# AIRI-Institute/nablaDFT

Measured on AMD Instinct MI355X. Metric: conformer-steps/sec (fwd+bwd) + MAE(E,F) vs CPU reference, higher is better.
Workload: dtype f32 (dense products >= 192 tiles: f32 values split exactly into 3 bf16 pieces, 6 MFMA piece products, f32 accumulate; non-finite operands give NaN where plain f32 gives inf); 1 GPU; PaiNN-OC (nablaDFT/painn_pyg, config/model/painn-oc.yaml: F=128 L=6 R=100 rc=5A K=100) energy+forces train step incl. neighbour list, L1+L2 loss, grad all-reduce, clip 5.0, AdamW lr 5e-4; synthetic ~42-atom drug-like conformers, 2048 conformers/GPU/step; conformers_per_gpu=2048, edges_last_step=1737976, parallelism=dp1

## Files before the change

### nabladft_amd/csrc/engine.hip

```cpp
#include <stdarg.h>
#include <stdlib.h>
#include <string.h>

#include "../../include/nablaq.h"
#include "common.h"

thread_local char nq_err_buf[512] = "";
int nq_fail(int code, const char* fmt, ...) {
  va_list ap;
  va_start(ap, fmt);
  vsnprintf(nq_err_buf, sizeof(nq_err_buf), fmt, ap);
  va_end(ap);
  return code;
}

#include <map>
#include <mutex>
#include <utility>
static std::mutex g_lds_mu;
static std::map<std::pair<int, const void*>, size_t> g_lds_granted;
int nq_dyn_lds(const void* kernel, size_t bytes) {
  int dev = 0;
  NQ_HIP(hipGetDevice(&dev));
  std::lock_guard<std::mutex> lock(g_lds_mu);
// ... 110 lines not shown
  W->GXH = take(2 * N * 3 * F); W->GH = take(2 * N * F);
  W->GBR = take(N * 3 * F);
  W->GPHI2 = take(2 * E * 3 * F);
  W->GEDGE = take((F / 64) * E * 4);
  W->GZO = take(2 * N * H); W->TMPW = take(N * H);
  W->GRHO = take(c->rbf_type ? 2 * E * R : 0); W->BCON = take(c->rbf_type ? E * R : 0);
  W->ROWCTR = take(5 * L * NQ_ROWCTR_INTS);
  W->SCHED = take(W->fused ? nq_molgw_sched_ints((int)E, (int)B) : 0);
  W->GWREC = take(W->fused ? nq_molgw_rec_floats((int)E, (int)B) : 0);
  W->GWPART = take(W->fused ? nq_molgw_part_floats((int)F, (int)B) : 0);
  size_t s = 0;
  auto mx = [&](size_t v) { if (v > s) s = v; };
  mx(nq_gemm_tn_scratch_floats(2 * N, 3 * F, F)); mx(nq_gemm_tn_scratch_floats(2 * N, F, 2 * F)); mx(nq_gemm_tn_scratch_floats(6 * N, 2 * F, F));
  mx(W->fused ? nq_gwr_scratch_floats((int)E, (int)F, (int)R) : nq_gemm_tn_scratch_floats(2 * E, 3 * F, R));
  if (W->fused) mx(nq_k0_sort_scratch_ints((int)E, (int)R));
  mx(nq_gemm_tn_scratch_floats(2 * N, F, F)); mx(nq_gemm_tn_scratch_floats(2 * N, H, F));
  mx(nq_colsum_scratch_floats(N > E ? N : E, 3 * F));
  if (c->rbf_type) { mx(nq_colsum_scratch_floats(E, R)); mx(nq_colsum_scratch_floats(E * R, 1)); }
  mx(nq_embed_grad_scratch_floats((int)N, (int)F, (int)T));
  W->scratch_floats = s;
  W->scratch = take(s);
  W->total_floats = o;
  (void)B;
}

enum { GW_PAIR_ROWS = 0, GW_MOLECULE = 1, GW_MIXED = 2 };
struct StepPlan {
  bool fused;
  int gw_mode, gw_cap;
  bool lite;
  bool fused_update;
  bool layer0;
  bool top_layer;
};
static StepPlan plan_step(const nq_painn_cfg* c, const nq_graph* g, bool want_forces) {
  auto env_on = [](const char* name) { const char* v = getenv(name); return v && v[0] == '1'; };
  StepPlan p{};
  p.fused = c->rbf_type == 0 && nq_filter_fits_lds(c->hidden_channels, c->num_rbf) && !env_on("NQ_NO_FUSED_FILTER");
  const char* cap = getenv("NQ_MOLGW_CAP");
  const int hw = nq_molgw_max_atoms();
  p.gw_cap = cap && atoi(cap) > 0 && atoi(cap) < hw ? atoi(cap) : hw;
  p.gw_mode = GW_PAIR_ROWS;
  if (p.fused && !env_on("NQ_NO_MOLGW") && nq_molgw_config_ok(c->hidden_channels, c->num_rbf) && g->max_mol_atoms > 0 && (env_on("NQ_MOLGW") || g->N >= 4096))
    p.gw_mode = g->max_mol_atoms <= p.gw_cap ? GW_MOLECULE : GW_MIXED;
  p.lite = p.fused && want_forces && !env_on("NQ_NO_LITE");
  p.fused_update = nq_updfuse_frag_floats(c->hidden_channels) > 0 && !env_on("NQ_NO_FUSED_UPDATE") && !nq_gemm_exact_f32_requested();
  p.layer0 = !env_on("NQ_NO_LAYER0");
  p.top_layer = !env_on("NQ_NO_TOPLAYER");
  return p;
}
static bool plan_fused(const nq_painn_cfg* c, int32_t N, int32_t E, int32_t B) {
  nq_graph g{};
  g.N = N; g.E = E; g.B = B;
  return plan_step(c, &g, false).fused;
}

struct StepRecord { nq_painn_cfg cfg; int32_t N, E, B, max_mol_atoms; StepPlan plan; };
static std::mutex g_plan_mu;
static std::map<const void*, StepRecord> g_plans;
static StepRecord g_last_plan;
static bool g_have_last_plan = false;
static void record_plan(const void* ws, const nq_painn_cfg* c, const nq_graph* g, const StepPlan& p) {
  std::lock_guard<std::mutex> lock(g_plan_mu);
  g_plans[ws] = StepRecord{*c, g->N, g->E, g->B, g->max_mol_atoms, p};
  g_last_plan = g_plans[ws]; g_have_last_plan = true;
}
static bool last_plan_for(const nq_painn_cfg* c, int32_t N, int32_t E, int32_t B, StepPlan* p) {
  std::lock_guard<std::mutex> lock(g_plan_mu);
  if (!g_have_last_plan || memcmp(&g_last_plan.cfg, c, sizeof(nq_painn_cfg)) != 0 || g_last_plan.N != N || g_last_plan.E != E || g_last_plan.B != B) return false;
  *p = g_last_plan.plan;
  return true;
}
static int recall_plan(const void* ws, const nq_painn_cfg* c, const nq_graph* g, StepPlan* p) {
  std::lock_guard<std::mutex> lock(g_plan_mu);
  auto it = g_plans.find(ws);
  if (it == g_plans.end()) return nq_fail(NQ_ERR_ARG, "nq_painn_backward: no forward call has prepared this workspace");
  const StepRecord& r = it->second;
  if (memcmp(&r.cfg, c, sizeof(nq_painn_cfg)) != 0 || r.N != g->N || r.E != g->E || r.B != g->B || r.max_mol_atoms != g->max_mol_atoms)
    return nq_fail(NQ_ERR_ARG, "nq_painn_backward: the last forward call on this workspace was made for a different model or batch");
  *p = r.plan;
  return NQ_OK;
}

static NqGraphView view_of(const nq_graph* g) {
  NqGraphView v;
  v.N = g->N; v.B = g->B; v.E = g->E;
  v.mol_ptr = g->mol_ptr; v.row_ptr = g->row_ptr; v.col = g->col; v.rev = g->rev;
  v.geom = reinterpret_cast<const float4*>(g->geom); v.z = g->z; v.atom_mol = g->atom_mol; v.lowptr = g->lowptr;
  return v;
}

static int check_common(const nq_painn_cfg* cfg, const nq_graph* g, const void* ws, size_t ws_bytes, bool fused, WsLayout* W, ParamLayout* P) {
  if (!cfg || !g || !ws) return nq_fail(NQ_ERR_ARG, "null argument");
  NQ_TRY(make_param_layout(cfg, P));
  if (g->N <= 0 || g->B <= 0) return nq_fail(NQ_ERR_ARG, "empty batch");
  if (g->E <= 0) return nq_fail(NQ_ERR_NO_EDGES, "batch has no edges within the cutoff");
  if ((reinterpret_cast<uintptr_t>(ws) & 15) != 0) return nq_fail(NQ_ERR_ARG, "workspace must be 16-byte aligned");
  make_ws_layout(cfg, g->N, g->E, g->B, fused, W);
  if (cfg->filter_mode != 0 && cfg->filter_mode != 1) return nq_fail(NQ_ERR_ARG, "filter_mode must be 0 (painn_pyg) or 1 (schnetpack)");
  if (cfg->filter_mode == 1 && !W->fused)
    return nq_fail(NQ_ERR_ARG, "filter_mode 1 (schnetpack) needs the fused-filter path: hidden_channels in {64,128,256} and WrT fitting the LDS");
  if (ws_bytes < W->total_floats * sizeof(float))
    return nq_fail(NQ_ERR_WORKSPACE, "workspace too small: %zu < %zu bytes", ws_bytes, W->total_floats * sizeof(float));
  return NQ_OK;
}

extern "C" {

int nq_abi_version(void) { return NQ_ABI_VERSION; }
int32_t nq_painn_molecule_lds_atoms(void) { return nq_molgw_max_atoms(); }

void nq_profile_enable(int32_t on) { nq_profile_on = on; }
int nq_profile_read2(char* names, int32_t name_stride, double* total_ms, int64_t* counts, double* flops, int32_t cap) {
  (void)hipDeviceSynchronize();
  std::vector<double> tot(g_prof_names.size(), 0.0), fl(g_prof_names.size(), 0.0);
  std::vector<long long> cnt(g_prof_names.size(), 0);
  for (auto& r : g_prof_recs) {
    float ms = 0.f;
    if (hipEventElapsedTime(&ms, r.a, r.b) == hipSuccess) { tot[r.name_id] += ms; cnt[r.name_id] += 1; fl[r.name_id] += r.flops; }
    (void)hipEventDestroy(r.a); (void)hipEventDestroy(r.b);
  }
  g_prof_recs.clear();
  int n = (int)g_prof_names.size();
  for (int i = 0; i < n && i < cap; ++i) {
    snprintf(names + (size_t)i * name_stride, name_stride, "%s", g_prof_names[i].c_str());
    total_ms[i] = tot[i]; counts[i] = cnt[i];
    if (flops) flops[i] = fl[i];
  }
  return n;
}
int nq_profile_read(char* names, int32_t name_stride, double* total_ms, int64_t* counts, int32_t cap) {
  return nq_profile_read2(names, name_stride, total_ms, counts, nullptr, cap);
}
const char* nq_last_error(void) { return nq_err_buf; }

int nq_graph_count(const float* pos, const int32_t* mol_ptr, int32_t N, int32_t B, int32_t max_mol_atoms, double cutoff,
                   int32_t max_neighbors, int32_t* deg, int32_t* lowdeg, int32_t* row_ptr, int32_t* lowptr, int32_t* E_host, void* stream) {
// ... 100 lines not shown
  else if (!strcmp(name, "e_atom")) { base = tangent ? W.te_atom : W.e_atom; rows = n; w = 1; dual = false; tangent = 0; }
  else if (!strcmp(name, "t_d")) { base = W.TD; rows = e; w = 1; dual = false; }
  else if (!strcmp(name, "t_r")) { base = W.TR; rows = e; w = 3; dual = false; }
  else if (!strcmp(name, "gedge")) { base = W.GEDGE; rows = (F / 64) * e; w = 4; dual = false; }
  else return nq_fail(NQ_ERR_ARG, "unknown workspace buffer '%s'", name);
#undef LAYER_OK
  if (tangent && !dual) return nq_fail(NQ_ERR_ARG, "buffer '%s' has no tangent half", name);
  *off = base + (tangent ? rows * w : 0);
  *count = rows * w;
  return NQ_OK;
}

int nq_painn_forward(const nq_painn_cfg* cfg, const float* params, const float* rbf_offsets, const nq_graph* graph, void* workspace,
                     size_t workspace_bytes, float* energy, float* forces, void* stream) {
  if (!cfg || !graph) return nq_fail(NQ_ERR_ARG, "null argument");
  const StepPlan plan = plan_step(cfg, graph, forces != nullptr);
  WsLayout W; ParamLayout P;
  NQ_TRY(check_common(cfg, graph, workspace, workspace_bytes, plan.fused, &W, &P));
  if (!params || !rbf_offsets || !energy) return nq_fail(NQ_ERR_ARG, "null argument");
  record_plan(workspace, cfg, graph, plan);
  hipStream_t st = (hipStream_t)stream;
  float* ws = (float*)workspace;
  const NqGraphView g = view_of(graph);
  const int N = g.N, E = g.E, F = cfg->hidden_channels, R = cfg->num_rbf, H = F / 2, L = cfg->num_layers;
  const size_t NF = (size_t)N * F;
  int* const rowctr0 = reinterpret_cast<int*>(ws + W.ROWCTR);
  NQ_HIP(hipMemsetAsync(rowctr0, 0, (size_t)2 * L * NQ_ROWCTR_INTS * sizeof(int), st));
  auto row_ctr = [&](int kind, int l) { return N >= 4096 ? rowctr0 + ((size_t)kind * L + l) * NQ_ROWCTR_INTS : (int*)nullptr; };

  NQ_TRY(nq_embed(st, g.z, params + P.emb, N, F, ws + W.X[0]));
  NQ_HIP(hipMemsetAsync(ws + W.X[0] + NF, 0, NF * sizeof(float), st));
  NQ_HIP(hipMemsetAsync(ws + W.V[0], 0, 6 * NF * sizeof(float), st));
  float* rho = ws + W.RHO2; float* drho = rho + (size_t)E * R;
  const bool lite_store = plan.lite;
  if (W.fused) {
    FilterArgs fa0;
    nq_make_filter_args(&fa0, nullptr, nullptr, rbf_offsets, ws + W.RW, R, cfg->cutoff, cfg->envelope_exponent, cfg->rbf_coeff, cfg->filter_mode);
    NQ_TRY(nq_rbf_window(st, g.geom, E, fa0, ws + W.RW));
    int* const sched = reinterpret_cast<int*>(ws + W.SCHED);
    if (plan.gw_mode != GW_PAIR_ROWS) NQ_TRY(nq_molgw_schedule(st, g, graph->dst, ws + W.RW, R, plan.gw_cap, sched, ws + W.GWREC));
    if (plan.gw_mode == GW_PAIR_ROWS) NQ_TRY(nq_k0_sort(st, ws + W.RW, E, R, reinterpret_cast<int*>(ws + W.ORDER), reinterpret_cast<int*>(ws + W.scratch), graph->dst, g.col));
    else if (plan.gw_mode == GW_MIXED)
      NQ_TRY(nq_k0_sort(st, ws + W.RW, E, R, reinterpret_cast<int*>(ws + W.ORDER), reinterpret_cast<int*>(ws + W.scratch), graph->dst, g.col, g.mol_ptr, g.atom_mol,
                        plan.gw_cap, sched + nq_molgw_sched_ints(E, g.B) - 1));
  } else {
    NQ_TRY(nq_rbf(st, g.geom, E, R, cfg->cutoff, cfg->envelope_exponent, cfg->rbf_coeff, rbf_offsets, rho, drho, cfg->rbf_type, params + P.basis));
  }

  for (int l = 0; l < L; ++l) {
    const WsLayer& y = W.lay[l]; const MsgP& mp = P.msg[l]; const UpdP& up = P.upd[l];
    NQ_TRY(nq_gemm_nt(st, ws + W.X[l], params + mp.W1, ws + y.Z1, params + mp.b1, ws + y.Hh, N, F, F, F, F, F, "W1"));
    NQ_TRY(nq_gemm_nt(st, ws + y.Hh, params + mp.W2, ws + y.XH, params + mp.b2, nullptr, N, 3 * F, F, F, F, 3 * F, "W2"));
    MsgArgs m{};
    m.g = g; m.F = F; m.X = ws + W.X[l]; m.V = ws + W.V[l]; m.XH = ws + y.XH; m.PHI = ws + y.PHI; m.PSI = ws + y.PSI;
    m.XM = ws + y.XM; m.VM = ws + y.VM;
    if (W.fused) {
      FilterArgs fa;
      NQ_TRY(nq_transpose(st, params + mp.Wr, 3 * F, R, ws + y.WRT));
      nq_make_filter_args(&fa, ws + y.WRT, params + mp.br, rbf_offsets, ws + W.RW, R, cfg->cutoff, cfg->envelope_exponent, cfg->rbf_coeff, cfg->filter_mode);
      fa.row_ctr = row_ctr(0, l);
      NQ_TRY(nq_msgf_fwd(st, m, fa, false, plan.layer0 && l == 0));
    } else {
      NQ_TRY(nq_gemm_nt(st, rho, params + mp.Wr, ws + y.PHI, params + mp.br, nullptr, E, 3 * F, R, R, R, 3 * F, "Wr"));
      NQ_TRY(nq_gemm_nt(st, drho, params + mp.Wr, ws + y.PSI, nullptr, nullptr, E, 3 * F, R, R, R, 3 * F, "Wr"));
      NQ_TRY(nq_msg_fwd(st, m, false));
    }
    UpdArgs u{};
    u.N = N; u.F = F; u.XM = ws + y.XM; u.VM = ws + y.VM; u.U = ws + y.UU; u.Y = ws + y.Y; u.S = ws + y.S; u.CAT = ws + y.CAT;
    u.X1 = ws + W.X[l + 1]; u.V1 = ws + W.V[l + 1];
    if (plan.fused_update) {
      NQ_TRY(nq_updfuse_presplit(st, params + up.U, params + up.V1, params + up.V2, F, ws + y.UFRAG));
      NQ_TRY(nq_upd_fused(st, u, ws + y.UFRAG, params + up.c1, params + up.c2, ws + y.ZQ, ws + y.Q));
      continue;
    }
    NQ_TRY(nq_gemm_nt(st, ws + y.VM, params + up.U, ws + y.UU, nullptr, nullptr, 3 * N, 2 * F, F, F, F, 2 * F, "U"));
    NQ_TRY(nq_upd_a(st, u, false));
    NQ_TRY(nq_gemm_nt(st, ws + y.CAT, params + up.V1, ws + y.ZQ, params + up.c1, ws + y.Q, N, F, 2 * F, 2 * F, 2 * F, F, "V1"));
    NQ_TRY(nq_gemm_nt(st, ws + y.Q, params + up.V2, ws + y.Y, params + up.c2, nullptr, N, 3 * F, F, F, F, 3 * F, "V2"));
    NQ_TRY(nq_upd_b(st, u, false));
  }
  NQ_TRY(nq_gemm_nt(st, ws + W.X[L], params + P.O1, ws + W.ZO, params + P.o1, nullptr, N, H, F, F, F, H, "O1"));
  ReadoutArgs r{};
  r.N = N; r.H = H; r.ZO = ws + W.ZO; r.w2 = params + P.w2; r.o2 = params + P.o2; r.e_atom = ws + W.e_atom;
  NQ_TRY(nq_readout(st, r, 0));
  NQ_TRY(nq_mol_sum(st, ws + W.e_atom, g.mol_ptr, g.B, energy));
  if (!forces) return NQ_OK;

  NQ_TRY(nq_atom_seeds(st, nullptr, g.atom_mol, N, ws + W.ge, nullptr));
  r.ge = ws + W.ge; r.GZO = ws + W.GZO;
  NQ_TRY(nq_readout_rev(st, r, false));
  float* gx_cur = lite_store ? ws + W.lay[L - 1].LGXA : ws + W.GX;
  NQ_TRY(nq_gemm_nn(st, ws + W.GZO, params + P.O1, gx_cur, N, H, F, H, F, F, 0, "O1"));
  float* gv_cur = lite_store ? ws + W.lay[L - 1].LGVA : ws + W.GVa; float* gv_oth = ws + W.GVb;
  if (lite_store || !plan.top_layer) NQ_HIP(hipMemsetAsync(gv_cur, 0, 3 * NF * sizeof(float), st));
  const int nwaves = F / 64;
  NQ_HIP(hipMemsetAsync(ws + W.GEDGE, 0, (size_t)nwaves * E * 4 * sizeof(float), st));
  for (int l = L - 1; l >= 0; --l) {
    const WsLayer& y = W.lay[l]; const MsgP& mp = P.msg[l]; const UpdP& up = P.upd[l];
    const bool top = plan.top_layer && l == L - 1;
    const int KY = top ? 2 * F : 3 * F;
    float* const GY = lite_store ? ws + y.LGY + 3 * NF : ws + W.GY;
    float* const GCAT = lite_store ? ws + y.LGCAT + 2 * NF : ws + W.GCAT;
    float* const GU = lite_store ? ws + y.LGU + 6 * NF : ws + W.GU;
    float* const GXH = lite_store ? ws + y.LGXH + 3 * NF : ws + W.GXH;
    float* const gx_msg = lite_store ? ws + y.LGXB : gx_cur;
    float* const gv_msg = lite_store ? ws + y.LGVB : gv_cur;
    float* const gx_next = lite_store ? (l > 0 ? ws + W.lay[l - 1].LGXA : ws + W.GX) : gx_cur;
    float* const gv_next = lite_store ? (l > 0 ? ws + W.lay[l - 1].LGVA : ws + W.GVb) : gv_oth;
    UpdRevArgs u{};
    u.N = N; u.F = F; u.U = ws + y.UU; u.Y = ws + y.Y; u.S = ws + y.S; u.CAT = ws + y.CAT;
    u.GX = gx_cur; u.GV = gv_cur; u.GY = GY; u.GCAT = GCAT; u.GU = GU;
    u.GX_out = lite_store ? gx_msg : nullptr;
    NQ_TRY(nq_upd_rev(st, u, 1, false, top));
    float* const GQ = lite_store ? ws + y.LGQ + NF : ws + W.GQ;
    if (lite_store) NQ_TRY(nq_gemm_nn_dsilu2(st, GY, params + up.V2, ws + y.LGQP, GQ, ws + y.ZQ, N, KY, F, "V2", 3 * F));
    else NQ_TRY(nq_gemm_nn_epi(st, GY, params + up.V2, GQ, N, KY, F, ws + y.ZQ, 0.f, 1.f, 1, "V2", 3 * F));
    NQ_TRY(nq_gemm_nn(st, GQ, params + up.V1, GCAT, N, F, 2 * F, F, 2 * F, 2 * F, 0, "V1"));
    NQ_TRY(nq_upd_rev(st, u, 2, false, top));
    if (lite_store && !top) NQ_TRY(nq_gemm_nn_epi(st, GU, params + up.U, gv_msg, 3 * N, 2 * F, F, gv_cur, 1.f, 0.f, 0, "U"));
    else NQ_TRY(nq_gemm_nn(st, GU, params + up.U, gv_msg, 3 * N, 2 * F, F, 2 * F, F, F, top ? 0 : 1, "U"));
    MsgRevArgs m{};
    m.g = g; m.F = F; m.V = ws + W.V[l]; m.XH = ws + y.XH; m.PHI = ws + y.PHI; m.PSI = ws + y.PSI;
    m.GX = gx_msg; m.GV = gv_msg; m.GXH = GXH; m.GV_out = gv_next; m.GEDGE = reinterpret_cast<float4*>(ws + W.GEDGE);
    if (W.fused) {
      FilterArgs fa;
      nq_make_filter_args(&fa, ws + y.WRT, params + mp.br, rbf_offsets, ws + W.RW, R, cfg->cutoff, cfg->envelope_exponent, cfg->rbf_coeff, cfg->filter_mode);
      fa.row_ctr = row_ctr(1, l);
      NQ_TRY(nq_msgf_rev(st, m, fa, false, true, plan.layer0 && l == 0));
    } else {
      NQ_TRY(nq_msg_rev(st, m, false));
    }
    float* const GH = lite_store ? ws + y.LGH + NF : ws + W.GH;
    if (lite_store) NQ_TRY(nq_gemm_nn_dsilu2(st, GXH, params + mp.W2, ws + y.LGHP, GH, ws + y.Z1, N, 3 * F, F, "W2"));
    else NQ_TRY(nq_gemm_nn_epi(st, GXH, params + mp.W2, GH, N, 3 * F, F, ws + y.Z1, 0.f, 1.f, 1, "W2"));
    if (plan.layer0 && l == 0) break;
    if (lite_store) {
      NQ_TRY(nq_gemm_nn_epi(st, GH, params + mp.W1, gx_next, N, F, F, gx_msg, 1.f, 0.f, 0, "W1"));
      gx_cur = gx_next; gv_cur = gv_next;
    } else {
      { float* t = gv_cur; gv_cur = gv_oth; gv_oth = t; }
      NQ_TRY(nq_gemm_nn(st, GH, params + mp.W1, gx_cur, N, F, F, F, F, F, 1, "W1"));
    }
  }
  NQ_TRY(nq_geom_rev(st, g, reinterpret_cast<const float4*>(ws + W.GEDGE), nwaves, forces));
  return NQ_OK;
}

struct SideStream {
  hipStream_t main = nullptr, side = nullptr;
  bool on = false;
  std::vector<hipEvent_t>* pool = nullptr;
  size_t used = 0;
  bool forked = false, joined = false;
  hipEvent_t last_read[8] = {};
  SideStream() = default;
  SideStream(const SideStream&) = delete;
  SideStream& operator=(const SideStream&) = delete;
  ~SideStream() { if (on && forked && !joined) join(); }
  hipEvent_t next() {
    if (used == pool->size()) { hipEvent_t e; if (hipEventCreateWithFlags(&e, hipEventDisableTiming) != hipSuccess) return nullptr; pool->push_back(e); }
    return (*pool)[used++];
  }
  hipStream_t fork() {
    if (!on) return main;
    hipEvent_t e = next();
    (void)hipEventRecord(e, main); (void)hipStreamWaitEvent(side, e, 0);
    forked = true; joined = false;
    return side;
  }
  void read_by_side(int buf) { if (on) { hipEvent_t e = next(); (void)hipEventRecord(e, side); last_read[buf] = e; } }
  void before_main_writes(int buf) { if (on && last_read[buf]) { (void)hipStreamWaitEvent(main, last_read[buf], 0); last_read[buf] = nullptr; } }
  void join() { if (on) { hipEvent_t e = next(); (void)hipEventRecord(e, side); (void)hipStreamWaitEvent(main, e, 0); joined = true; } }
};
enum { SB_GY = 0, SB_GQ, SB_GU, SB_GXH, SB_GH, SB_GPHI, SB_GBR };
struct SidePool { hipStream_t side = nullptr; std::vector<hipEvent_t> events; };
static std::mutex g_side_mu;
static std::map<std::pair<int, hipStream_t>, SidePool*> g_side_pools;
static void side_stream_init(SideStream& s, hipStream_t main, int n_atoms) {
  s.main = main;
  const char* env = getenv("NQ_SIDE_STREAM");
  const bool want = env && (env[0] == '0' || env[0] == '1') ? env[0] == '1' : (n_atoms <= 16384 || !nq_profile_on);
  if (!want) return;
  int dev = 0;
  if (hipGetDevice(&dev) != hipSuccess) return;
  std::lock_guard<std::mutex> lock(g_side_mu);
  SidePool*& pool = g_side_pools[std::make_pair(dev, main)];
  if (!pool) {
    SidePool* p = new SidePool();
    if (hipStreamCreateWithFlags(&p->side, hipStreamNonBlocking) != hipSuccess) { delete p; return; }
    pool = p;
  }
  s.side = pool->side; s.pool = &pool->events; s.on = true;
}

static int painn_backward_impl(const nq_painn_cfg* cfg, const float* params, const float* rbf_offsets, const nq_graph* graph, void* workspace,
                               size_t workspace_bytes, const float* grad_energy, const float* grad_forces, float* grad_params, void* stream,
                               bool seeded, const float* seed_x, const float* seed_vec, void* const* layer_events = nullptr) {
  if (!cfg || !graph || !workspace) return nq_fail(NQ_ERR_ARG, "null argument");
  StepPlan plan;
  NQ_TRY(recall_plan(workspace, cfg, graph, &plan));
  WsLayout W; ParamLayout P;
  NQ_TRY(check_common(cfg, graph, workspace, workspace_bytes, plan.fused, &W, &P));
  if (!params || !grad_params || !rbf_offsets) return nq_fail(NQ_ERR_ARG, "null argument");
  hipStream_t st = (hipStream_t)stream;
  float* ws = (float*)workspace;
  float* gp = grad_params;
  float* scr = ws + W.scratch;
  const NqGraphView g = view_of(graph);
  const int N = g.N, E = g.E, F = cfg->hidden_channels, R = cfg->num_rbf, H = F / 2, L = cfg->num_layers, T = cfg->num_elements;
  const size_t NF = (size_t)N * F;
  int* const rowctr0 = reinterpret_cast<int*>(ws + W.ROWCTR);
  NQ_HIP(hipMemsetAsync(rowctr0 + (size_t)2 * L * NQ_ROWCTR_INTS, 0, (size_t)3 * L * NQ_ROWCTR_INTS * sizeof(int), st));
  auto row_ctr = [&](int kind, int l) { return N >= 4096 ? rowctr0 + ((size_t)kind * L + l) * NQ_ROWCTR_INTS : (int*)nullptr; };

  const size_t NH = (size_t)N * H;
  ReadoutArgs r{};
  r.N = N; r.H = H; r.ZO = ws + W.ZO; r.TZO = ws + W.ZO + NH; r.w2 = params + P.w2; r.o2 = params + P.o2;
  r.e_atom = ws + W.e_atom; r.te_atom = ws + W.te_atom;
  if (seeded) {
    auto zero = [&](size_t off, size_t n) { return hipMemsetAsync(ws + off, 0, n * sizeof(float), st); };
    for (int l = 0; l <= L; ++l) { NQ_HIP(zero(W.X[l] + NF, NF)); NQ_HIP(zero(W.V[l] + 3 * NF, 3 * NF)); }
    for (int l = 0; l < L; ++l) {
      const WsLayer& y = W.lay[l];
      NQ_HIP(zero(y.Z1 + NF, NF)); NQ_HIP(zero(y.Hh + NF, NF)); NQ_HIP(zero(y.XH + 3 * NF, 3 * NF)); NQ_HIP(zero(y.XM + NF, NF));
      NQ_HIP(zero(y.VM + 3 * NF, 3 * NF)); NQ_HIP(zero(y.UU + 6 * NF, 6 * NF)); NQ_HIP(zero(y.S + NF, NF)); NQ_HIP(zero(y.CAT + 2 * NF, 2 * NF));
      NQ_HIP(zero(y.ZQ + NF, NF)); NQ_HIP(zero(y.Q + NF, NF)); NQ_HIP(zero(y.Y + 3 * NF, 3 * NF));
    }
    NQ_HIP(zero(W.TD, E)); NQ_HIP(zero(W.TR, 3 * (size_t)E)); NQ_HIP(zero(W.ZO + (size_t)N * H, (size_t)N * H)); NQ_HIP(zero(W.te_atom, N));
  } else {
  if (grad_forces) NQ_TRY(nq_negate(st, grad_forces, ws + W.pos_dot, 3L * N));
  else NQ_HIP(hipMemsetAsync(ws + W.pos_dot, 0, 3 * (size_t)N * sizeof(float), st));
  NQ_TRY(nq_geom_tan(st, g, graph->dst, ws + W.pos_dot, ws + W.TD, ws + W.TR));
  for (int l = 0; l < L; ++l) {
    const WsLayer& y = W.lay[l]; const MsgP& mp = P.msg[l]; const UpdP& up = P.upd[l];
    float* TZ1 = ws + y.Z1 + NF; float* TH = ws + y.Hh + NF; float* TXH = ws + y.XH + 3 * NF;
    if (plan.layer0 && l == 0) {
      NQ_HIP(hipMemsetAsync(TZ1, 0, NF * sizeof(float), st));
      NQ_HIP(hipMemsetAsync(TH, 0, NF * sizeof(float), st));
      NQ_HIP(hipMemsetAsync(TXH, 0, 3 * NF * sizeof(float), st));
    } else {
      NQ_TRY(nq_gemm_nt_dsilu(st, ws + W.X[l] + NF, params + mp.W1, TZ1, TH, ws + y.Z1, N, F, F, "W1"));
      NQ_TRY(nq_gemm_nt(st, TH, params + mp.W2, TXH, nullptr, nullptr, N, 3 * F, F, F, F, 3 * F, "W2"));
    }
    MsgArgs m{};
    m.g = g; m.F = F; m.X = ws + W.X[l]; m.V = ws + W.V[l]; m.XH = ws + y.XH; m.PHI = ws + y.PHI; m.PSI = ws + y.PSI;
    m.TX = ws + W.X[l] + NF; m.TV = ws + W.V[l] + 3 * NF; m.TXH = TXH; m.TD = ws + W.TD; m.TR = ws + W.TR;
    m.TXM = ws + y.XM + NF; m.TVM = ws + y.VM + 3 * NF;
    if (W.fused) {
      FilterArgs fa;
      nq_make_filter_args(&fa, ws + y.WRT, params + mp.br, rbf_offsets, ws + W.RW, R, cfg->cutoff, cfg->envelope_exponent, cfg->rbf_coeff, cfg->filter_mode);
      fa.row_ctr = row_ctr(2, l);
      NQ_TRY(nq_msgf_fwd(st, m, fa, true, plan.layer0 && l == 0));
    } else {
      NQ_TRY(nq_msg_fwd(st, m, true));
    }
    UpdArgs u{};
    u.N = N; u.F = F; u.XM = ws + y.XM; u.VM = ws + y.VM; u.U = ws + y.UU; u.Y = ws + y.Y; u.S = ws + y.S; u.CAT = ws + y.CAT;
    u.TXM = ws + y.XM + NF; u.TVM = ws + y.VM + 3 * NF; u.TU = ws + y.UU + 6 * NF; u.TY = ws + y.Y + 3 * NF;
    u.TS = ws + y.S + NF; u.TCAT = ws + y.CAT + 2 * NF; u.TX1 = ws + W.X[l + 1] + NF; u.TV1 = ws + W.V[l + 1] + 3 * NF;
    float* TZQ = ws + y.ZQ + NF; float* TQ = ws + y.Q + NF;
    NQ_TRY(nq_gemm_nt(st, ws + y.VM + 3 * NF, params + up.U, ws + y.UU + 6 * NF, nullptr, nullptr, 3 * N, 2 * F, F, F, F, 2 * F, "U"));
    NQ_TRY(nq_upd_a(st, u, true));
    NQ_TRY(nq_gemm_nt_dsilu(st, ws + y.CAT + 2 * NF, params + up.V1, TZQ, TQ, ws + y.ZQ, N, F, 2 * F, "V1"));
    NQ_TRY(nq_gemm_nt(st, TQ, params + up.V2, ws + y.Y + 3 * NF, nullptr, nullptr, N, 3 * F, F, F, F, 3 * F, "V2"));
    NQ_TRY(nq_upd_b(st, u, true));
  }
  NQ_TRY(nq_gemm_nt(st, ws + W.X[L] + NF, params + P.O1, ws + W.ZO + NH, nullptr, nullptr, N, H, F, F, F, H, "O1"));
  r.N = N; r.H = H; r.ZO = ws + W.ZO; r.TZO = ws + W.ZO + NH; r.w2 = params + P.w2; r.o2 = params + P.o2;
  r.e_atom = ws + W.e_atom; r.te_atom = ws + W.te_atom;
  NQ_TRY(nq_readout(st, r, 1));

  }
  if (grad_energy) NQ_TRY(nq_atom_seeds(st, grad_energy, g.atom_mol, N, ws + W.ge, ws + W.gte));
  else {
    NQ_HIP(hipMemsetAsync(ws + W.ge, 0, (size_t)N * sizeof(float), st));
    NQ_TRY(nq_atom_seeds(st, nullptr, g.atom_mol, N, ws + W.gte, nullptr));
  }
  if (seeded) NQ_HIP(hipMemsetAsync(ws + W.gte, 0, (size_t)N * sizeof(float), st));
  r.ge = ws + W.ge; r.gte = ws + W.gte; r.GZO = ws + W.GZO; r.GTZO = ws + W.GZO + NH; r.TMPW = ws + W.TMPW;
  NQ_TRY(nq_readout_rev(st, r, true));
  const bool lite = plan.lite && !seeded;
  SideStream ss;
  if (plan.gw_mode != GW_MIXED) side_stream_init(ss, st, N);
  hipStream_t sd = ss.fork();
  NQ_TRY(nq_colsum(sd, ws + W.TMPW, N, H, H, gp + P.w2, scr));
  NQ_TRY(nq_colsum(sd, ws + W.ge, N, 1, 1, gp + P.o2, scr));
  NQ_TRY(nq_gemm_tn(sd, ws + W.GZO, ws + W.X[L], gp + P.O1, 2L * N, H, F, H, F, scr, "O1", gp + P.o1, N));
  NQ_TRY(nq_gemm_nn(st, ws + W.GZO, params + P.O1, ws + W.GX, lite ? N : 2 * N, H, F, H, F, F, 0, "O1"));
  float* gv_cur = ws + W.GVa; float* gv_oth = ws + W.GVb;
  const bool top_layer = plan.top_layer && !seeded;
  if (!top_layer) NQ_HIP(hipMemsetAsync(gv_cur, 0, (lite ? 3 : 6) * NF * sizeof(float), st));
  if (seeded) {
    if (seed_x) NQ_TRY(nq_axpy(st, seed_x, ws + W.GX, (long)NF));
    if (seed_vec) NQ_HIP(hipMemcpyAsync(gv_cur, seed_vec, 3 * NF * sizeof(float), hipMemcpyDeviceToDevice, st));
  }
  float* gphi = ws + W.GPHI2; float* gpsi = gphi + (size_t)E * 3 * F;
  const bool molgw = plan.gw_mode != GW_PAIR_ROWS, mixed = plan.gw_mode == GW_MIXED;
  const int* const sched = reinterpret_cast<const int*>(ws + W.SCHED);
  const int* const n_big_pairs = sched + nq_molgw_sched_ints(E, g.B) - 1;
  if (molgw) NQ_TRY(nq_molgw_geometry(st, g, ws + W.RW, ws + W.TD, ws + W.TR, sched, ws + W.GWREC));
  if (mixed) NQ_HIP(hipMemsetAsync(ws + W.GBR, 0, 3 * NF * sizeof(float), st));
  for (int l = L - 1; l >= 0; --l) {
    const WsLayer& y = W.lay[l]; const MsgP& mp = P.msg[l]; const UpdP& up = P.upd[l];
    const bool top = top_layer && l == L - 1;
    const bool l0 = plan.layer0 && l == 0;
    float* const GYs = lite ? ws + y.LGY : ws + W.GY;
    float* const GCATs = lite ? ws + y.LGCAT : ws + W.GCAT;
    float* const GUs = lite ? ws + y.LGU : ws + W.GU;
    float* const GXHs = lite ? ws + y.LGXH : ws + W.GXH;
    float* const GQs = lite ? ws + y.LGQ : ws + W.GQ;
    float* const GHs = lite ? ws + y.LGH : ws + W.GH;
    UpdRevArgs u{};
    u.N = N; u.F = F; u.U = ws + y.UU; u.Y = ws + y.Y; u.S = ws + y.S; u.CAT = ws + y.CAT;
    u.TU = ws + y.UU + 6 * NF; u.TY = ws + y.Y + 3 * NF; u.TS = ws + y.S + NF; u.TCAT = ws + y.CAT + 2 * NF;
    u.GX = ws + W.GX; u.GTX = lite ? ws + y.LGXA : ws + W.GX + NF; u.GV = gv_cur; u.GTV = lite ? ws + y.LGVA : gv_cur + 3 * NF;
    u.GY = GYs; u.GTY = GYs + 3 * NF; u.GCAT = GCATs; u.GTCAT = GCATs + 2 * NF;
    u.GU = GUs; u.GTU = GUs + 6 * NF;
    u.lite = lite ? 1 : 0;
    ss.before_main_writes(SB_GY);
    NQ_TRY(nq_upd_rev(st, u, 1, true, top));
    sd = ss.fork();
    NQ_TRY(nq_gemm_tn(sd, GYs, ws + y.Q, gp + up.V2, 2L * N, 3 * F, F, 3 * F, F, scr, "V2", gp + up.c2, N));
    ss.read_by_side(SB_GY);
    ss.before_main_writes(SB_GQ);
    NQ_TRY(nq_gemm_nn(st, GYs, params + up.V2, GQs, lite ? N : 2 * N, top ? 2 * F : 3 * F, F, 3 * F, F, F, 0, "V2"));
    NQ_TRY(nq_silu_rev(st, ws + y.ZQ, ws + y.ZQ + NF, GQs, lite ? ws + y.LGQP : GQs + NF, (long)NF, true, lite));
    sd = ss.fork();
    NQ_TRY(nq_gemm_tn(sd, GQs, ws + y.CAT, gp + up.V1, 2L * N, F, 2 * F, F, 2 * F, scr, "V1", gp + up.c1, N));
    ss.read_by_side(SB_GQ);
    NQ_TRY(nq_gemm_nn(st, GQs, params + up.V1, GCATs, lite ? N : 2 * N, F, 2 * F, F, 2 * F, 2 * F, 0, "V1"));
    ss.before_main_writes(SB_GU);
    NQ_TRY(nq_upd_rev(st, u, 2, true, top));
    sd = ss.fork();
    NQ_TRY(nq_gemm_tn(sd, GUs, ws + y.VM, gp + up.U, 6L * N, 2 * F, F, 2 * F, F, scr, "U"));
    ss.read_by_side(SB_GU);
    NQ_TRY(nq_gemm_nn(st, GUs, params + up.U, gv_cur, lite ? 3 * N : 6 * N, 2 * F, F, 2 * F, F, F, top ? 0 : 1, "U"));
    MsgRevArgs m{};
    m.g = g; m.F = F; m.V = ws + W.V[l]; m.XH = ws + y.XH; m.PHI = ws + y.PHI; m.PSI = ws + y.PSI;
    m.TV = ws + W.V[l] + 3 * NF; m.TXH = ws + y.XH + 3 * NF; m.TD = ws + W.TD; m.TR = ws + W.TR;
    m.GX = ws + W.GX; m.GV = gv_cur; m.GTX = lite ? ws + y.LGXB : ws + W.GX + NF; m.GTV = lite ? ws + y.LGVB : gv_cur + 3 * NF;
    m.GXH = GXHs; m.GTXH = GXHs + 3 * NF; m.GV_out = gv_oth; m.GTV_out = gv_oth + 3 * NF;
    m.lite = lite ? 1 : 0;
    m.GPHI = gphi; m.GPSI = gpsi; m.GBR = ws + W.GBR;
    ss.before_main_writes(SB_GXH); ss.before_main_writes(SB_GPHI); ss.before_main_writes(SB_GBR);
    if (W.fused) {
      FilterArgs fa;
      nq_make_filter_args(&fa, ws + y.WRT, params + mp.br, rbf_offsets, ws + W.RW, R, cfg->cutoff, cfg->envelope_exponent, cfg->rbf_coeff, cfg->filter_mode);
      fa.row_ctr = row_ctr(3, l);
      m.mol_cap = plan.gw_cap;
      m.row_filter = mixed ? 1 : 0;
      NQ_TRY(nq_msgf_rev(st, m, fa, true, !molgw, l0));
      if (mixed) {
        m.row_filter = 2;
        fa.row_ctr = row_ctr(4, l);
        NQ_TRY(nq_msgf_rev(st, m, fa, true, true));
        NQ_TRY(nq_gwr_sorted(st, gphi, gpsi, ws + W.RW, reinterpret_cast<const int*>(ws + W.ORDER), E / 2, F, R, gp + mp.Wr, scr, 3, n_big_pairs));
        NQ_TRY(nq_colsum(st, ws + W.GBR, N, 3 * F, 3 * F, gp + mp.br, scr));
      }
      if (molgw)
        NQ_TRY(nq_gwr_mol(st, g, F, R, plan.gw_cap, m.XH, m.V, m.TXH, m.TV, m.GX, m.GV, m.GTX, m.GTV, sched, ws + W.GWREC, ws + W.GWPART, gp + mp.Wr, gp + mp.br, mixed, l0));
    } else {
      NQ_TRY(nq_msg_rev(st, m, true));
    }
    { float* t = gv_cur; gv_cur = gv_oth; gv_oth = t; }
    sd = ss.fork();
    if (W.fused && !molgw) NQ_TRY(nq_gwr_sorted(sd, gphi, gpsi, ws + W.RW, reinterpret_cast<const int*>(ws + W.ORDER), E / 2, F, R, gp + mp.Wr, scr));
    else if (!W.fused) NQ_TRY(nq_gemm_tn(sd, gphi, ws + W.RHO2, gp + mp.Wr, 2L * E, 3 * F, R, 3 * F, R, scr, "Wr"));
    if (cfg->rbf_type)
      NQ_TRY(nq_gemm_nn(st, gphi, params + mp.Wr, ws + W.GRHO, 2 * E, 3 * F, R, 3 * F, R, R, l == L - 1 ? 0 : 1, "Wr"));
    if (!molgw) NQ_TRY(nq_colsum(sd, ws + W.GBR, N, 3 * F, 3 * F, gp + mp.br, scr));
    NQ_TRY(nq_gemm_tn(sd, GXHs, ws + y.Hh, gp + mp.W2, l0 ? (long)N : 2L * N, 3 * F, F, 3 * F, F, scr, "W2", gp + mp.b2, N));
    ss.read_by_side(SB_GPHI); ss.read_by_side(SB_GBR); ss.read_by_side(SB_GXH);
    ss.before_main_writes(SB_GH);
    NQ_TRY(nq_gemm_nn(st, GXHs, params + mp.W2, GHs, lite ? N : 2 * N, 3 * F, F, 3 * F, F, F, 0, "W2"));
    NQ_TRY(nq_silu_rev(st, ws + y.Z1, ws + y.Z1 + NF, GHs, lite ? ws + y.LGHP : GHs + NF, (long)NF, true, lite));
    sd = ss.fork();
    NQ_TRY(nq_gemm_tn(sd, GHs, ws + W.X[l], gp + mp.W1, l0 ? (long)N : 2L * N, F, F, F, F, scr, "W1", gp + mp.b1, N));
    ss.read_by_side(SB_GH);
    NQ_TRY(nq_gemm_nn(st, GHs, params + mp.W1, ws + W.GX, lite ? N : 2 * N, F, F, F, F, F, 1, "W1"));
    if (layer_events && layer_events[L - 1 - l]) NQ_HIP(hipEventRecord((hipEvent_t)layer_events[L - 1 - l], ss.on ? ss.side : st));
  }
  ss.join();
  NQ_TRY(nq_embed_grad(st, g.z, ws + W.GX, N, F, T, gp + P.emb, scr));
  if (cfg->rbf_type) {
    NQ_TRY(nq_rbf_param_grad(st, g.geom, E, R, cfg->cutoff, cfg->envelope_exponent, rbf_offsets, cfg->rbf_type, params + P.basis, ws + W.GRHO, ws + W.BCON));
    if (cfg->rbf_type == 1) NQ_TRY(nq_colsum(st, ws + W.BCON, E, R, R, gp + P.basis, scr));
    else NQ_TRY(nq_colsum(st, ws + W.BCON, (long)E * R, 1, 1, gp + P.basis, scr));
  }
  return NQ_OK;
}

int nq_painn_backward(const nq_painn_cfg* cfg, const float* params, const float* rbf_offsets, const nq_graph* graph, void* workspace,
                      size_t workspace_bytes, const float* grad_energy, const float* grad_forces, float* grad_params, void* stream) {
  return painn_backward_impl(cfg, params, rbf_offsets, graph, workspace, workspace_bytes, grad_energy, grad_forces, grad_params, stream, false, nullptr,
                             nullptr);
}
int nq_painn_backward_events(const nq_painn_cfg* cfg, const float* params, const float* rbf_offsets, const nq_graph* graph, void* workspace,
                             size_t workspace_bytes, const float* grad_energy, const float* grad_forces, float* grad_params, void* const* layer_events_host,
                             void* stream) {
  return painn_backward_impl(cfg, params, rbf_offsets, graph, workspace, workspace_bytes, grad_energy, grad_forces, grad_params, stream, false, nullptr,
                             nullptr, layer_events_host);
}
int nq_painn_layer_param_ranges(const nq_painn_cfg* cfg, int64_t* ranges_host) {
  ParamLayout P;
  if (!cfg || !ranges_host) return nq_fail(NQ_ERR_ARG, "null argument");
  NQ_TRY(make_param_layout(cfg, &P));
  const int L = cfg->num_layers;
  for (int l = 0; l < L; ++l) {
    const size_t m0 = P.msg[l].W1, m1 = l + 1 < L ? P.msg[l + 1].W1 : P.upd[0].U;
    const size_t u0 = P.upd[l].U, u1 = l + 1 < L ? P.upd[l + 1].U : P.O1;
    ranges_host[4 * l + 0] = (int64_t)m0; ranges_host[4 * l + 1] = (int64_t)(m1 - m0);
    ranges_host[4 * l + 2] = (int64_t)u0; ranges_host[4 * l + 3] = (int64_t)(u1 - u0);
  }
  ranges_host[4 * L + 0] = (int64_t)P.O1; ranges_host[4 * L + 1] = (int64_t)(P.total - P.O1);
  ranges_host[4 * L + 2] = 0; ranges_host[4 * L + 3] = (int64_t)P.msg[0].W1;
  return NQ_OK;
// ... 28 lines not shown
```

Before: 51690 conformer-steps/s.

## Overlap molecule-tiled filter weight-grad and schedule build on a side stream

When the per-molecule weight-gradient path is used with the lite backward, two pieces of work move to a side stream: the molecule schedule build in the forward pass and the nq_gwr_mol weight-gradient kernel in each backward layer. To avoid a write-after-read hazard on the GX gradient buffer, the W1 input-gradient GEMM now writes into a second GX buffer through an epilogue that adds the current one, and the two buffers swap each layer. Cross-stream hazards are tracked with new buffer slots (GV, GX0, GX1). The aim is to hide the weight-gradient kernel behind the main backward chain. The cost is extra event traffic, and there is a correctness risk if main-stream forward kernels read the schedule before the final join.

```diff
diff --git a/nabladft_amd/csrc/engine.hip b/nabladft_amd/csrc/engine.hip
--- a/nabladft_amd/csrc/engine.hip
+++ b/nabladft_amd/csrc/engine.hip
@@ -166,6 +166,7 @@
   bool fused_update;
   bool layer0;
   bool top_layer;
+  bool gw_side;
 };
 static StepPlan plan_step(const nq_painn_cfg* c, const nq_graph* g, bool want_forces) {
   auto env_on = [](const char* name) { const char* v = getenv(name); return v && v[0] == '1'; };
@@ -181,6 +182,8 @@
   p.fused_update = nq_updfuse_frag_floats(c->hidden_channels) > 0 && !env_on("NQ_NO_FUSED_UPDATE") && !nq_gemm_exact_f32_requested();
   p.layer0 = !env_on("NQ_NO_LAYER0");
   p.top_layer = !env_on("NQ_NO_TOPLAYER");
+  const char* gws = getenv("NQ_GW_SIDE");
+  p.gw_side = p.gw_mode == GW_MOLECULE && p.lite && !(gws && gws[0] == '0');
   return p;
 }
 static bool plan_fused(const nq_painn_cfg* c, int32_t N, int32_t E, int32_t B) {
@@ -237,6 +240,54 @@
   if (ws_bytes < W->total_floats * sizeof(float))
     return nq_fail(NQ_ERR_WORKSPACE, "workspace too small: %zu < %zu bytes", ws_bytes, W->total_floats * sizeof(float));
   return NQ_OK;
+}
+
+struct SideStream {
+  hipStream_t main = nullptr, side = nullptr;
+  bool on = false;
+  std::vector<hipEvent_t>* pool = nullptr;
+  size_t used = 0;
+  bool forked = false, joined = false;
+  hipEvent_t last_read[12] = {};
+  SideStream() = default;
+  SideStream(const SideStream&) = delete;
+  SideStream& operator=(const SideStream&) = delete;
+  ~SideStream() { if (on && forked && !joined) join(); }
+  hipEvent_t next() {
+    if (used == pool->size()) { hipEvent_t e; if (hipEventCreateWithFlags(&e, hipEventDisableTiming) != hipSuccess) return nullptr; pool->push_back(e); }
+    return (*pool)[used++];
+  }
+  hipStream_t fork() {
+    if (!on) return main;
+    hipEvent_t e = next();
+    (void)hipEventRecord(e, main); (void)hipStreamWaitEvent(side, e, 0);
+    forked = true; joined = false;
+    return side;
+  }
+  void read_by_side(int buf) { if (on) { hipEvent_t e = next(); (void)hipEventRecord(e, side); last_read[buf] = e; } }
+  void before_main_writes(int buf) { if (on && last_read[buf]) { (void)hipStreamWaitEvent(main, last_read[buf], 0); last_read[buf] = nullptr; } }
+  void join() { if (on) { hipEvent_t e = next(); (void)hipEventRecord(e, side); (void)hipStreamWaitEvent(main, e, 0); joined = true; } }
+};
+enum { SB_GY = 0, SB_GQ, SB_GU, SB_GXH, SB_GH, SB_GPHI, SB_GBR, SB_GV, SB_GX0, SB_GX1, SB_COUNT };
+static_assert(SB_COUNT <= 12, "SideStream::last_read");
+struct SidePool { hipStream_t side = nullptr; std::vector<hipEvent_t> events; };
+static std::mutex g_side_mu;
+static std::map<std::pair<int, hipStream_t>, SidePool*> g_side_pools;
+static void side_stream_init(SideStream& s, hipStream_t main, int n_atoms) {
+  s.main = main;
+  const char* env = getenv("NQ_SIDE_STREAM");
+  const bool want = env && (env[0] == '0' || env[0] == '1') ? env[0] == '1' : (n_atoms <= 16384 || !nq_profile_on);
+  if (!want) return;
+  int dev = 0;
+  if (hipGetDevice(&dev) != hipSuccess) return;
+  std::lock_guard<std::mutex> lock(g_side_mu);
+  SidePool*& pool = g_side_pools[std::make_pair(dev, main)];
+  if (!pool) {
+    SidePool* p = new SidePool();
+    if (hipStreamCreateWithFlags(&p->side, hipStreamNonBlocking) != hipSuccess) { delete p; return; }
+    pool = p;
+  }
+  s.side = pool->side; s.pool = &pool->events; s.on = true;
 }
 
 extern "C" {
@@ -403,13 +454,15 @@
   NQ_HIP(hipMemsetAsync(ws + W.X[0] + NF, 0, NF * sizeof(float), st));
   NQ_HIP(hipMemsetAsync(ws + W.V[0], 0, 6 * NF * sizeof(float), st));
   float* rho = ws + W.RHO2; float* drho = rho + (size_t)E * R;
+  SideStream ss;
+  if (plan.gw_side) side_stream_init(ss, st, N);
   const bool lite_store = plan.lite;
   if (W.fused) {
     FilterArgs fa0;
     nq_make_filter_args(&fa0, nullptr, nullptr, rbf_offsets, ws + W.RW, R, cfg->cutoff, cfg->envelope_exponent, cfg->rbf_coeff, cfg->filter_mode);
     NQ_TRY(nq_rbf_window(st, g.geom, E, fa0, ws + W.RW));
     int* const sched = reinterpret_cast<int*>(ws + W.SCHED);
-    if (plan.gw_mode != GW_PAIR_ROWS) NQ_TRY(nq_molgw_schedule(st, g, graph->dst, ws + W.RW, R, plan.gw_cap, sched, ws + W.GWREC));
+    if (plan.gw_mode != GW_PAIR_ROWS) NQ_TRY(nq_molgw_schedule(plan.gw_side ? ss.fork() : st, g, graph->dst, ws + W.RW, R, plan.gw_cap, sched, ws + W.GWREC));
     if (plan.gw_mode == GW_PAIR_ROWS) NQ_TRY(nq_k0_sort(st, ws + W.RW, E, R, reinterpret_cast<int*>(ws + W.ORDER), reinterpret_cast<int*>(ws + W.scratch), graph->dst, g.col));
     else if (plan.gw_mode == GW_MIXED)
       NQ_TRY(nq_k0_sort(st, ws + W.RW, E, R, reinterpret_cast<int*>(ws + W.ORDER), reinterpret_cast<int*>(ws + W.scratch), graph->dst, g.col, g.mol_ptr, g.atom_mol,
@@ -455,7 +508,7 @@
   r.N = N; r.H = H; r.ZO = ws + W.ZO; r.w2 = params + P.w2; r.o2 = params + P.o2; r.e_atom = ws + W.e_atom;
   NQ_TRY(nq_readout(st, r, 0));
   NQ_TRY(nq_mol_sum(st, ws + W.e_atom, g.mol_ptr, g.B, energy));
-  if (!forces) return NQ_OK;
+  if (!forces) { if (ss.forked) ss.join(); return NQ_OK; }
 
   NQ_TRY(nq_atom_seeds(st, nullptr, g.atom_mol, N, ws + W.ge, nullptr));
   r.ge = ws + W.ge; r.GZO = ws + W.GZO;
@@ -514,54 +567,8 @@
     }
   }
   NQ_TRY(nq_geom_rev(st, g, reinterpret_cast<const float4*>(ws + W.GEDGE), nwaves, forces));
+  if (ss.forked) ss.join();
   return NQ_OK;
-}
-
-struct SideStream {
-  hipStream_t main = nullptr, side = nullptr;
-  bool on = false;
-  std::vector<hipEvent_t>* pool = nullptr;
-  size_t used = 0;
-  bool forked = false, joined = false;
-  hipEvent_t last_read[8] = {};
-  SideStream() = default;
-  SideStream(const SideStream&) = delete;
-  SideStream& operator=(const SideStream&) = delete;
-  ~SideStream() { if (on && forked && !joined) join(); }
-  hipEvent_t next() {
-    if (used == pool->size()) { hipEvent_t e; if (hipEventCreateWithFlags(&e, hipEventDisableTiming) != hipSuccess) return nullptr; pool->push_back(e); }
-    return (*pool)[used++];
-  }
-  hipStream_t fork() {
-    if (!on) return main;
-    hipEvent_t e = next();
-    (void)hipEventRecord(e, main); (void)hipStreamWaitEvent(side, e, 0);
-    forked = true; joined = false;
-    return side;
-  }
-  void read_by_side(int buf) { if (on) { hipEvent_t e = next(); (void)hipEventRecord(e, side); last_read[buf] = e; } }
-  void before_main_writes(int buf) { if (on && last_read[buf]) { (void)hipStreamWaitEvent(main, last_read[buf], 0); last_read[buf] = nullptr; } }
-  void join() { if (on) { hipEvent_t e = next(); (void)hipEventRecord(e, side); (void)hipStreamWaitEvent(main, e, 0); joined = true; } }
-};
-enum { SB_GY = 0, SB_GQ, SB_GU, SB_GXH, SB_GH, SB_GPHI, SB_GBR };
-struct SidePool { hipStream_t side = nullptr; std::vector<hipEvent_t> events; };
-static std::mutex g_side_mu;
-static std::map<std::pair<int, hipStream_t>, SidePool*> g_side_pools;
-static void side_stream_init(SideStream& s, hipStream_t main, int n_atoms) {
-  s.main = main;
-  const char* env = getenv("NQ_SIDE_STREAM");
-  const bool want = env && (env[0] == '0' || env[0] == '1') ? env[0] == '1' : (n_atoms <= 16384 || !nq_profile_on);
-  if (!want) return;
-  int dev = 0;
-  if (hipGetDevice(&dev) != hipSuccess) return;
-  std::lock_guard<std::mutex> lock(g_side_mu);
-  SidePool*& pool = g_side_pools[std::make_pair(dev, main)];
-  if (!pool) {
-    SidePool* p = new SidePool();
-    if (hipStreamCreateWithFlags(&p->side, hipStreamNonBlocking) != hipSuccess) { delete p; return; }
-    pool = p;
-  }
-  s.side = pool->side; s.pool = &pool->events; s.on = true;
 }
 
 static int painn_backward_impl(const nq_painn_cfg* cfg, const float* params, const float* rbf_offsets, const nq_graph* graph, void* workspace,
@@ -588,6 +595,10 @@
   ReadoutArgs r{};
   r.N = N; r.H = H; r.ZO = ws + W.ZO; r.TZO = ws + W.ZO + NH; r.w2 = params + P.w2; r.o2 = params + P.o2;
   r.e_atom = ws + W.e_atom; r.te_atom = ws + W.te_atom;
+  SideStream ss;
+  if (plan.gw_mode != GW_MIXED) side_stream_init(ss, st, N);
+  const bool gw_side = plan.gw_side && !seeded && ss.on;
+  const int* const sched = reinterpret_cast<const int*>(ws + W.SCHED);
   if (seeded) {
     auto zero = [&](size_t off, size_t n) { return hipMemsetAsync(ws + off, 0, n * sizeof(float), st); };
     for (int l = 0; l <= L; ++l) { NQ_HIP(zero(W.X[l] + NF, NF)); NQ_HIP(zero(W.V[l] + 3 * NF, 3 * NF)); }
@@ -651,23 +662,22 @@
   r.ge = ws + W.ge; r.gte = ws + W.gte; r.GZO = ws + W.GZO; r.GTZO = ws + W.GZO + NH; r.TMPW = ws + W.TMPW;
   NQ_TRY(nq_readout_rev(st, r, true));
   const bool lite = plan.lite && !seeded;
-  SideStream ss;
-  if (plan.gw_mode != GW_MIXED) side_stream_init(ss, st, N);
   hipStream_t sd = ss.fork();
   NQ_TRY(nq_colsum(sd, ws + W.TMPW, N, H, H, gp + P.w2, scr));
   NQ_TRY(nq_colsum(sd, ws + W.ge, N, 1, 1, gp + P.o2, scr));
   NQ_TRY(nq_gemm_tn(sd, ws + W.GZO, ws + W.X[L], gp + P.O1, 2L * N, H, F, H, F, scr, "O1", gp + P.o1, N));
-  NQ_TRY(nq_gemm_nn(st, ws + W.GZO, params + P.O1, ws + W.GX, lite ? N : 2 * N, H, F, H, F, F, 0, "O1"));
+  float* gx_cur = ws + W.GX; float* gx_oth = ws + W.GX + NF;
+  int gx_slot = SB_GX0, gx_oth_slot = SB_GX1;
+  NQ_TRY(nq_gemm_nn(st, ws + W.GZO, params + P.O1, gx_cur, lite ? N : 2 * N, H, F, H, F, F, 0, "O1"));
   float* gv_cur = ws + W.GVa; float* gv_oth = ws + W.GVb;
   const bool top_layer = plan.top_layer && !seeded;
   if (!top_layer) NQ_HIP(hipMemsetAsync(gv_cur, 0, (lite ? 3 : 6) * NF * sizeof(float), st));
   if (seeded) {
-    if (seed_x) NQ_TRY(nq_axpy(st, seed_x, ws + W.GX, (long)NF));
+    if (seed_x) NQ_TRY(nq_axpy(st, seed_x, gx_cur, (long)NF));
     if (seed_vec) NQ_HIP(hipMemcpyAsync(gv_cur, seed_vec, 3 * NF * sizeof(float), hipMemcpyDeviceToDevice, st));
   }
   float* gphi = ws + W.GPHI2; float* gpsi = gphi + (size_t)E * 3 * F;
   const bool molgw = plan.gw_mode != GW_PAIR_ROWS, mixed = plan.gw_mode == GW_MIXED;
-  const int* const sched = reinterpret_cast<const int*>(ws + W.SCHED);
   const int* const n_big_pairs = sched + nq_molgw_sched_ints(E, g.B) - 1;
   if (molgw) NQ_TRY(nq_molgw_geometry(st, g, ws + W.RW, ws + W.TD, ws + W.TR, sched, ws + W.GWREC));
   if (mixed) NQ_HIP(hipMemsetAsync(ws + W.GBR, 0, 3 * NF * sizeof(float), st));
@@ -684,7 +694,7 @@
     UpdRevArgs u{};
     u.N = N; u.F = F; u.U = ws + y.UU; u.Y = ws + y.Y; u.S = ws + y.S; u.CAT = ws + y.CAT;
     u.TU = ws + y.UU + 6 * NF; u.TY = ws + y.Y + 3 * NF; u.TS = ws + y.S + NF; u.TCAT = ws + y.CAT + 2 * NF;
-    u.GX = ws + W.GX; u.GTX = lite ? ws + y.LGXA : ws + W.GX + NF; u.GV = gv_cur; u.GTV = lite ? ws + y.LGVA : gv_cur + 3 * NF;
+    u.GX = gx_cur; u.GTX = lite ? ws + y.LGXA : ws + W.GX + NF; u.GV = gv_cur; u.GTV = lite ? ws + y.LGVA : gv_cur + 3 * NF;
     u.GY = GYs; u.GTY = GYs + 3 * NF; u.GCAT = GCATs; u.GTCAT = GCATs + 2 * NF;
     u.GU = GUs; u.GTU = GUs + 6 * NF;
     u.lite = lite ? 1 : 0;
@@ -709,11 +719,12 @@
     MsgRevArgs m{};
     m.g = g; m.F = F; m.V = ws + W.V[l]; m.XH = ws + y.XH; m.PHI = ws + y.PHI; m.PSI = ws + y.PSI;
     m.TV = ws + W.V[l] + 3 * NF; m.TXH = ws + y.XH + 3 * NF; m.TD = ws + W.TD; m.TR = ws + W.TR;
-    m.GX = ws + W.GX; m.GV = gv_cur; m.GTX = lite ? ws + y.LGXB : ws + W.GX + NF; m.GTV = lite ? ws + y.LGVB : gv_cur + 3 * NF;
+    m.GX = gx_cur; m.GV = gv_cur; m.GTX = lite ? ws + y.LGXB : ws + W.GX + NF; m.GTV = lite ? ws + y.LGVB : gv_cur + 3 * NF;
     m.GXH = GXHs; m.GTXH = GXHs + 3 * NF; m.GV_out = gv_oth; m.GTV_out = gv_oth + 3 * NF;
     m.lite = lite ? 1 : 0;
     m.GPHI = gphi; m.GPSI = gpsi; m.GBR = ws + W.GBR;
     ss.before_main_writes(SB_GXH); ss.before_main_writes(SB_GPHI); ss.before_main_writes(SB_GBR);
+    ss.before_main_writes(SB_GV);
     if (W.fused) {
       FilterArgs fa;
       nq_make_filter_args(&fa, ws + y.WRT, params + mp.br, rbf_offsets, ws + W.RW, R, cfg->cutoff, cfg->envelope_exponent, cfg->rbf_coeff, cfg->filter_mode);
@@ -728,8 +739,11 @@
         NQ_TRY(nq_gwr_sorted(st, gphi, gpsi, ws + W.RW, reinterpret_cast<const int*>(ws + W.ORDER), E / 2, F, R, gp + mp.Wr, scr, 3, n_big_pairs));
         NQ_TRY(nq_colsum(st, ws + W.GBR, N, 3 * F, 3 * F, gp + mp.br, scr));
       }
-      if (molgw)
-        NQ_TRY(nq_gwr_mol(st, g, F, R, plan.gw_cap, m.XH, m.V, m.TXH, m.TV, m.GX, m.GV, m.GTX, m.GTV, sched, ws + W.GWREC, ws + W.GWPART, gp + mp.Wr, gp + mp.br, mixed, l0));
+      if (molgw) {
+        NQ_TRY(nq_gwr_mol(gw_side ? ss.fork() : st, g, F, R, plan.gw_cap, m.XH, m.V, m.TXH, m.TV, m.GX, m.GV, m.GTX, m.GTV, sched, ws + W.GWREC, ws + W.GWPART,
+                          gp + mp.Wr, gp + mp.br, mixed, l0));
+        if (gw_side) { ss.read_by_side(SB_GV); ss.read_by_side(gx_slot); }
+      }
     } else {
       NQ_TRY(nq_msg_rev(st, m, true));
     }
@@ -748,11 +762,18 @@
     sd = ss.fork();
     NQ_TRY(nq_gemm_tn(sd, GHs, ws + W.X[l], gp + mp.W1, l0 ? (long)N : 2L * N, F, F, F, F, scr, "W1", gp + mp.b1, N));
     ss.read_by_side(SB_GH);
-    NQ_TRY(nq_gemm_nn(st, GHs, params + mp.W1, ws + W.GX, lite ? N : 2 * N, F, F, F, F, F, 1, "W1"));
+    if (gw_side) {
+      ss.before_main_writes(gx_oth_slot);
+      NQ_TRY(nq_gemm_nn_epi(st, GHs, params + mp.W1, gx_oth, N, F, F, gx_cur, 1.f, 0.f, 0, "W1"));
+      { float* t = gx_cur; gx_cur = gx_oth; gx_oth = t; }
+      { const int t = gx_slot; gx_slot = gx_oth_slot; gx_oth_slot = t; }
+    } else {
+      NQ_TRY(nq_gemm_nn(st, GHs, params + mp.W1, gx_cur, lite ? N : 2 * N, F, F, F, F, F, 1, "W1"));
+    }
     if (layer_events && layer_events[L - 1 - l]) NQ_HIP(hipEventRecord((hipEvent_t)layer_events[L - 1 - l], ss.on ? ss.side : st));
   }
   ss.join();
-  NQ_TRY(nq_embed_grad(st, g.z, ws + W.GX, N, F, T, gp + P.emb, scr));
+  NQ_TRY(nq_embed_grad(st, g.z, gx_cur, N, F, T, gp + P.emb, scr));
   if (cfg->rbf_type) {
     NQ_TRY(nq_rbf_param_grad(st, g.geom, E, R, cfg->cutoff, cfg->envelope_exponent, rbf_offsets, cfg->rbf_type, params + P.basis, ws + W.GRHO, ws + W.BCON));
     if (cfg->rbf_type == 1) NQ_TRY(nq_colsum(st, ws + W.BCON, E, R, R, gp + P.basis, scr));
```

Result: no change. 52190 conformer-steps/s (median of 6 runs) (+1.0%).
